# shibatch/rectdetect

Hardware: AMD Instinct MI355X
Metric: 1920x1080 frames/sec (higher is better)
Workload: dtype u8/i32/f32 (bit-exact integer + IEEE f32 stencil path)

## Files before the change

### rectdetect_amd/csrc/rd_k_poly.hip

```cpp
#include "rd_device.h"
#include "rd_kernels.h"

#include "rd_poly_scratch.h"
#include "rd_tidy_tile.h"

namespace {

using namespace rd;
using rdk::PolyScratch;
using rdk::PolyFrame;
#define RD_FRAME const PolyFrame &FRM = FRS.f[blockIdx.z]; const PolyScratch &s = FRM.ps

inline int cdiv(int a, int b) { return (a + b - 1) / b; }
const dim3 block2(64, 4);
inline dim3 grid2(int iw, int ih) { return dim3(cdiv(iw, 64), cdiv(ih, 4)); }
#define RD_XY const int x = blockIdx.x * 64 + threadIdx.x, y = blockIdx.y * 4 + threadIdx.y
#define SPARSE_GRID 512
#define SPARSE_LOOP(i, cnt) for (int i = blockIdx.x * blockDim.x + threadIdx.x; i < (cnt); i += gridDim.x * blockDim.x)

struct ls_rec { float x0, y0, x1, y1; int startIndex, endIndex, leftPtr, rightPtr, startCount, endCount, maxDist, polyid, npix, level; };
struct lsx_rec { long long mx00, mx01, mx11, my0, my1; short dx, dy, vx, vy; int d2, pad; };

typedef unsigned long long u64;
#define PT_M 6
#define TB_OUT (64 - 2 * PT_M)

__global__ __launch_bounds__(256) void k_mask_bits(const rdk::PolyFrames FRS, int iw, int ih, int wpr) {
  RD_FRAME;
  const int x = blockIdx.x * 64 + threadIdx.x, y = blockIdx.y * 4 + threadIdx.y;
  if (y >= ih) return;
  const bool in = x < iw;
  const int v = FRM.in[in ? y * iw + x : 0];
  const u64 m = __ballot(in && v != 0);
  u64 q = 0;
  if (FRM.ring_src != nullptr) {
    const bool ring = in && (y <= 1 || y >= ih - 2 || x <= 1 || x >= iw - 2);
    const int g = ring ? FRM.ring_src[y * iw + x] : 0;
    q = __ballot(g != 0);
  }
  if (threadIdx.x == 0) { s.sb[y * wpr + blockIdx.x] = m; s.rb[y * wpr + blockIdx.x] = q; }
}

__device__ __forceinline__ bitrow br_lane(bitrow a, int src_lane) {
  const unsigned a0 = (unsigned)a.lo, a1 = (unsigned)(a.lo >> 32), a2 = (unsigned)a.hi, a3 = (unsigned)(a.hi >> 32);
  const unsigned b0 = __shfl(a0, src_lane), b1 = __shfl(a1, src_lane), b2 = __shfl(a2, src_lane), b3 = __shfl(a3, src_lane);
  return br((u64)b0 | ((u64)b1 << 32), (u64)b2 | ((u64)b3 << 32));
}

__global__ __launch_bounds__(256) void k_tidy_bits(const rdk::PolyFrames FRS, int ring_const, int iw, int ih, int wpr) {
  RD_FRAME;
  const u64 *__restrict__ SB = FRM.in_bits != nullptr ? FRM.in_bits : s.sb;
  const u64 *__restrict__ RB = (FRM.in_bits == nullptr && FRM.ring_src != nullptr) ? s.rb : nullptr;
  if (blockIdx.x == 0 && blockIdx.y == 0 && threadIdx.x == 0) s.csync[0] = s.csync[0] + 1;
  const int lane = threadIdx.x & 63, wx = blockIdx.x * 4 + (threadIdx.x >> 6);
  if (wx >= wpr) return;
  constexpr int R = 64;
  const int x0 = wx * 64, y0 = blockIdx.y * TB_OUT;
  const int r = lane, y = y0 - PT_M + r;
  const bool yin = y >= 0 && y < ih;
  bitrow M = br(0, 0), RG = br(0, 0);
  if (yin) {
    const u64 *row = SB + (size_t)y * wpr + wx;
    const u64 W = wx > 0 ? row[-1] : 0ull, C = row[0], E = wx + 1 < wpr ? row[1] : 0ull;
    M = br((W >> 58) | (C << 6), (C >> 58) | (E << 6));
    if (RB != nullptr) {
      const u64 *rr = RB + (size_t)y * wpr + wx;
      const u64 W2 = wx > 0 ? rr[-1] : 0ull, C2 = rr[0], E2w = wx + 1 < wpr ? rr[1] : 0ull;
      RG = br((W2 >> 58) | (C2 << 6), (C2 >> 58) | (E2w << 6));
    }
  }
  const int b0 = PT_M - x0;
// ... 59 lines not shown
  const int lane = threadIdx.x & 63, y = blockIdx.x * 4 + (threadIdx.x >> 6);
  if (y >= ih) return;
  int run = 0;
  for (int w0 = 0; w0 < wpr; w0 += 64) {
    const int i = w0 + lane;
    const int c = i < wpr ? __popcll(s.tb[(size_t)y * wpr + i]) : 0;
    int inc = c;
#pragma unroll
    for (int o = 1; o < 64; o <<= 1) { const int t = __shfl_up(inc, o); if (lane >= o) inc += t; }
    if (i < wpr) s.pw[(size_t)y * wpr + i] = run + inc - c;
    run += __shfl(inc, 63);
  }
  if (lane == 0) s.rowsum[y] = run;
}

__device__ __forceinline__ int px_rank(const PolyScratch &s, int wpr, int qx, int qy) {
  const size_t wi = (size_t)qy * wpr + (qx >> 6);
  const u64 w = s.tb[wi];
  const int b = qx & 63;
  if (!((w >> b) & 1ull)) return -1;
  return s.rowbase[qy] + s.pw[wi] + __popcll(w & ((1ull << b) - 1ull));
}

#define CS_ROWS_PER_BLOCK 8
__global__ __launch_bounds__(256) void k_chain_scatter(const rdk::PolyFrames FRS, int iw, int ih, int wpr) {
  RD_FRAME;
  __shared__ int part[256];
  __shared__ int base[CS_ROWS_PER_BLOCK + 1];
  const int tid = threadIdx.x, ya = blockIdx.x * CS_ROWS_PER_BLOCK;
  int acc = 0;
  for (int i = tid; i < ya; i += 256) acc += s.rowsum[i];
  part[tid] = acc;
  __syncthreads();
  for (int o = 128; o > 0; o >>= 1) { if (tid < o) part[tid] += part[tid + o]; __syncthreads(); }
  if (tid == 0) {
    int run = part[0];
    for (int j = 0; j < CS_ROWS_PER_BLOCK; j++) {
      base[j] = run;
      if (ya + j < ih) { s.rowbase[ya + j] = run; run += s.rowsum[ya + j]; }
    }
    base[CS_ROWS_PER_BLOCK] = run;
    if (ya + CS_ROWS_PER_BLOCK >= ih) s.ctr[0] = run;
  }
  __syncthreads();
  for (int t = tid; t < CS_ROWS_PER_BLOCK * wpr; t += 256) {
    const int j = t / wpr, wx = t - j * wpr, y = ya + j;
    if (y >= ih) break;
    u64 w = s.tb[(size_t)y * wpr + wx];
    int rank = base[j] + s.pw[(size_t)y * wpr + wx];
    const int p = y * iw + wx * 64;
    while (w) {
      const int b = __ffsll((long long)w) - 1;
      w &= w - 1;
      s.pos[rank] = p + b; s.lab[rank] = rank; s.ends[rank] = 0;
      rank++;
    }
  }
}

#define CP_PER_BLOCK 8192
#define CP_K (CP_PER_BLOCK / 256)
__device__ __forceinline__ unsigned long long cp_word(unsigned gen, unsigned status, unsigned value) { return ((unsigned long long)(gen & 0xffffffu) << 40) | ((unsigned long long)status << 38) | value; }
template <int MODE>
__global__ __launch_bounds__(256) void k_compact1(const rdk::PolyFrames FRS, int n, int nblk, int size_thre, int init_ls) {
  RD_FRAME;
  static_assert(MODE == 1 || MODE == 2, "two call sites");
  int *__restrict__ pos = MODE == 2 ? s.live : nullptr;
  int *__restrict__ rank1 = MODE == 1 ? s.rootid : nullptr;
  const int *nptr = s.ctr;
  int *cnt = MODE == 1 ? s.ctr + 1 : s.ctr + 24;
  unsigned long long *state = s.cstate + (size_t)MODE * nblk;
  const int *genp = s.csync;
  ls_rec *ls = (MODE == 2 && init_ls) ? (ls_rec *)FRM.lslist : nullptr;
  if (MODE == 2 && ls != nullptr && blockIdx.x == 0 && threadIdx.x == 0) {
    ls_rec z = {};
    ls[0] = z;
    s.segaux[0] = -1; s.segaux[1] = 0x7fffffff;
    for (int k = 2; k < 24; k++) s.ctr[k] = 0;
    s.ctr[25] = 0;
  }
  __shared__ int wcount[CP_K * 4 + 1];
  __shared__ int s_excl;
  const int tid = threadIdx.x, lane = tid & 63, w = tid >> 6;
  const int b = blockIdx.x;
  if (nptr) n = *nptr;
  if (b * CP_PER_BLOCK >= n) { if (b == 0 && tid == 0 && cnt) *cnt = 0; return; }
  const unsigned gen = (unsigned)*genp;
  unsigned on = 0;
  if (MODE == 1) {
    int l[CP_K], sz[CP_K];
#pragma unroll
    for (int k = 0; k < CP_K; k++) { const int i = b * CP_PER_BLOCK + k * 256 + tid; const int q = i < n ? i : 0; l[k] = s.lab2[q]; sz[k] = s.size[q]; }
#pragma unroll
    for (int k = 0; k < CP_K; k++) { const int i = b * CP_PER_BLOCK + k * 256 + tid; if (i < n && l[k] == i && sz[k] > size_thre) on |= 1u << k; }
  } else {
    int l[CP_K];
#pragma unroll
    for (int k = 0; k < CP_K; k++) { const int i = b * CP_PER_BLOCK + k * 256 + tid; l[k] = s.lab2[i < n ? i : 0]; }
#pragma unroll
    for (int k = 0; k < CP_K; k++) l[k] = l[k] >= 0 ? s.rootid[l[k]] : 0;
#pragma unroll
    for (int k = 0; k < CP_K; k++) { const int i = b * CP_PER_BLOCK + k * 256 + tid; if (i < n) { s.id[i] = l[k]; if (l[k] != 0) on |= 1u << k; } }
  }
#pragma unroll
  for (int k = 0; k < CP_K; k++) { const unsigned long long m = __ballot((on >> k) & 1u); if (lane == 0) wcount[k * 4 + w] = __popcll(m); }
  __syncthreads();
  if (w == 0) {
    constexpr int CP_E = (CP_K * 4 + 63) / 64;
    int e[CP_E], c = 0;
#pragma unroll
    for (int q = 0; q < CP_E; q++) { e[q] = lane * CP_E + q < CP_K * 4 ? wcount[lane * CP_E + q] : 0; c += e[q]; }
    int inc = c;
#pragma unroll
    for (int o = 1; o < 64; o <<= 1) { const int t = __shfl_up(inc, o); if (lane >= o) inc += t; }
    int run = inc - c;
#pragma unroll
    for (int q = 0; q < CP_E; q++) { if (lane * CP_E + q < CP_K * 4) wcount[lane * CP_E + q] = run; run += e[q]; }
    const int total = __shfl(inc, 63);
    if (lane == 0) __hip_atomic_store(&state[b], cp_word(gen, b == 0 ? 2u : 1u, (unsigned)total), __ATOMIC_RELAXED, __HIP_MEMORY_SCOPE_AGENT);
    int excl = 0;
    for (int j = b - 1; j >= 0; j -= 64) {
      const int idx = j - lane;
      unsigned long long st;
      bool ready;
      int spins = 0;
      do {
        st = idx >= 0 ? __hip_atomic_load(&state[idx], __ATOMIC_RELAXED, __HIP_MEMORY_SCOPE_AGENT) : cp_word(gen, 2u, 0u);
        ready = (unsigned)(st >> 40) == (gen & 0xffffffu) && ((st >> 38) & 3ull) != 0ull;
        if (++spins > (1 << 24)) abort();
      } while (!__all(ready));
      const unsigned long long pm = __ballot(((st >> 38) & 3ull) == 2ull);
      const int upto = pm ? __ffsll((long long)pm) - 1 : 63;
      int v = lane <= upto ? (int)(st & 0x3fffffffffull) : 0;
#pragma unroll
      for (int o = 32; o > 0; o >>= 1) v += __shfl_xor(v, o);
      excl += v;
      if (pm) break;
    }
    if (lane == 0) {
      s_excl = excl;
      if (b > 0) __hip_atomic_store(&state[b], cp_word(gen, 2u, (unsigned)(excl + total)), __ATOMIC_RELAXED, __HIP_MEMORY_SCOPE_AGENT);
      if ((b + 1) * CP_PER_BLOCK >= n && cnt) *cnt = excl + total;
    }
  }
  __syncthreads();
  const int excl = s_excl;
#pragma unroll
  for (int k = 0; k < CP_K; k++) {
    const int i = b * CP_PER_BLOCK + k * 256 + tid;
    const bool o = (on >> k) & 1u;
    const unsigned long long m = __ballot(o);
    if (i >= n) continue;
    const int rank = excl + wcount[k * 4 + w] + __popcll(m & ((1ull << lane) - 1ull));
    if (o) { if (pos) pos[rank] = i; if (rank1) rank1[i] = rank + 1; }
  }
}

__global__ void k_chain_union(const rdk::PolyFrames FRS, int iw, int wpr) {
  RD_FRAME;
  const int cnt = s.ctr[0];
  SPARSE_LOOP(i, cnt) {
    const int p = s.pos[i];
    const int py = p / iw, px = p - py * iw;
    int nb[8], deg = 0;
#pragma unroll
    for (int k = 0; k < 8; k++) nb[k] = px_rank(s, wpr, px + nbr_dx(k), py + nbr_dy(k));
#pragma unroll
    for (int k = 0; k < 8; k++) { s.nbr[i * 8 + k] = nb[k]; deg += nb[k] >= 0; }
    s.flag2[i] = deg;
#pragma unroll
    for (int k = 0; k < 8; k++) if (nb[k] >= 0 && nb[k] < i) uf_union(s.lab, i, nb[k]);
  }
}

__global__ void k_flatten(const rdk::PolyFrames FRS, int which) {
  RD_FRAME;
  int *lab = which == 0 ? s.lab : s.lab2;
  int *ends = which == 0 ? s.ends : nullptr;
  const int *deg = s.flag2;
  int *size = which == 0 ? nullptr : s.size;
  const int cnt = s.ctr[0];
  for (int i0 = (blockIdx.x * blockDim.x + threadIdx.x) & ~63; i0 < cnt; i0 += gridDim.x * blockDim.x) {
    const int lane = threadIdx.x & 63, i = i0 + lane;
    int r = -1;
    if (i < cnt) {
      const int l = lab[i];
      r = l;
      if (l >= 0) { r = uf_find(lab, l); if (r != l) lab[i] = r; }
      if (ends != nullptr && deg[i] == 1) atomicAdd(&ends[r], 1);
    }
    if (size != nullptr) {
      const int prev = __shfl_up(r, 1);
      const bool start = lane == 0 || prev != r;
      const unsigned long long after = __ballot(start) & ~((2ull << lane) - 1ull);
      if (start && r >= 0) atomicAdd(&size[r], (after ? __ffsll((long long)after) - 1 : 64) - lane);
    }
  }
}

__global__ void k_find_ends0(const rdk::PolyFrames FRS) {
  RD_FRAME;
  const int cnt = s.ctr[0];
  SPARSE_LOOP(i, cnt) {
    int nb[8], lb[8], eb[8];
#pragma unroll
    for (int k = 0; k < 8; k++) nb[k] = s.nbr[i * 8 + k];
    const int li = s.lab[i], ei = s.ends[i];
#pragma unroll
    for (int k = 0; k < 8; k++) { const int j = nb[k] >= 0 ? nb[k] : i; lb[k] = s.lab[j]; eb[k] = s.ends[j]; }
    int a = i, b = i;
    const bool me = !(li == i && ei == 0);
    s.alive[i] = me ? 1 : 0;
    if (me) {
      int found = 0;
#pragma unroll
      for (int k = 0; k < 8; k++) {
        const bool living = nb[k] >= 0 && !(lb[k] == nb[k] && eb[k] == 0);
        if (living && found == 0) { a = nb[k]; found = 1; }
        else if (living && found == 1) { b = nb[k]; found = 2; }
      }
    }
    s.nx[0][i] = a; s.pv[0][i] = b;
  }
}

__global__ void k_find_ends0_flags(const rdk::PolyFrames FRS) {
  RD_FRAME;
  const int cnt = s.ctr[0];
  SPARSE_LOOP(i, cnt) {
    int f = 0;
    if (s.alive[i]) {
      const int a = s.nx[0][i], b = s.pv[0][i];
      if (a != i && s.nx[0][a] == i) f |= 1;
      if (b != i && s.pv[0][b] == i) f |= 2;
    }
    s.flag[i] = f;
  }
}

__global__ void k_find_ends1(const rdk::PolyFrames FRS, int page, int final) {
  RD_FRAME;
  const int cnt = s.ctr[0];
  const int *ni = s.nx[page], *pi = s.pv[page];
  int *no = s.nx[page ^ 1], *po = s.pv[page ^ 1];
  const int *fin = page == 0 ? s.flag : s.flag2;
  int *fout = page == 0 ? s.flag2 : s.flag;
  SPARSE_LOOP(i, cnt) {
    if (!s.alive[i]) { no[i] = i; po[i] = i; fout[i] = fin[i]; if (final) { s.num[0][i] = 0; s.link[0][i] = -1; } continue; }
    const int f0 = fin[i];
    bool revn = page == 0 ? (f0 & 1) != 0 : (f0 & 4) != 0;
    bool revp = page == 0 ? (f0 & 2) != 0 : (f0 & 8) != 0;
    int nn = ni[i], pp = pi[i];
    for (int h = 0; h < 8; h++) {
      const int nn2 = revn ? pi[nn] : ni[nn];
      const int pp2 = revp ? ni[pp] : pi[pp];
      int nf = fin[nn], pf = fin[pp];
      if (page != 0) { nf >>= 2; pf >>= 2; }
      revn = revn ? ((nf & 2) == 0) : ((nf & 1) != 0);
      revp = revp ? ((pf & 1) == 0) : ((pf & 2) != 0);
      nn = nn2; pp = pp2;
    }
    no[i] = nn; po[i] = pp;
    int f = f0;
    if (page == 0) { f &= 3; f |= revn ? 4 : 0; f |= revp ? 8 : 0; }
    else { f &= (3 << 2); f |= revn ? 1 : 0; f |= revp ? 2 : 0; }
    fout[i] = f;
    if (final) {
      int nb[8], al[8];
#pragma unroll
      for (int k = 0; k < 8; k++) nb[k] = s.nbr[i * 8 + k];
#pragma unroll
      for (int k = 0; k < 8; k++) al[k] = s.alive[nb[k] >= 0 ? nb[k] : i];
      int a = i, b = i, found = 0;
#pragma unroll
      for (int k = 0; k < 8; k++) {
        const bool living = nb[k] >= 0 && al[k] != 0;
        if (living && found == 0) { a = nb[k]; found = 1; }
        else if (living && found == 1) { b = nb[k]; found = 2; }
      }
      const int lk = nn < pp ? a : b;
      s.num[0][i] = lk == i ? 0 : 1; s.link[0][i] = lk;
    }
  }
}

__global__ void k_number(const rdk::PolyFrames FRS, int src, int init_sub) {
  RD_FRAME;
  const int cnt = s.ctr[0];
  const int *ni = s.num[src], *li = s.link[src];
  int *no = s.num[src ^ 1], *lo_ = s.link[src ^ 1];
  SPARSE_LOOP(i, cnt) {
    int n = ni[i], l = li[i];
    if (l != -1) {
      bool ok = true;
      for (int h = 0; h < 32; h++) {
        if (l < 0) { ok = false; break; }
        n += ni[l];
        l = li[l];
      }
      n = ok ? n : 0;
      l = ok ? l : -1;
    }
    no[i] = n;
    lo_[i] = l;
    if (init_sub) { s.lab2[i] = n == 0 ? -1 : i; s.size[i] = 0; s.rootid[i] = 0; }
  }
}

__global__ void k_sub_union(const rdk::PolyFrames FRS) {
  RD_FRAME;
  const int *__restrict__ number = s.num[1];
  const int cnt = s.ctr[0];
  SPARSE_LOOP(i, cnt) {
    const int a = number[i];
    if (a == 0) continue;
#pragma unroll
    for (int k = 0; k < 8; k++) {
      const int j = s.nbr[i * 8 + k];
      if (j < 0 || j > i) continue;
      const int b = number[j];
      if (b == 0) continue;
      const int d = a > b ? a - b : b - a;
      if (d <= 1) uf_union(s.lab2, i, j);
    }
  }
}

#define FITS(g, bytes) ((g) >= 0 && (long long)(bytes) > (long long)((g) + 1) * 56ll)

__device__ __forceinline__ void d_seg_clear(const rdk::PolyFrames &FRS, int lsbytes) {
  RD_FRAME;
  ls_rec *ls = (ls_rec *)FRM.lslist;
  const int K = s.ctr[1];
  const int maxrec = lsbytes / 56;
  SPARSE_LOOP(g, K + 1) {
    if (g >= maxrec) continue;
    ls_rec z = {};
    ls[g] = z;
    s.segaux[2 * g] = -1;
    s.segaux[2 * g + 1] = 0x7fffffff;
  }
  if (blockIdx.x == 0 && threadIdx.x == 0) { for (int k = 2; k < 24; k++) s.ctr[k] = 0; s.ctr[25] = 0; }
}
__global__ void k_seg_clear(const rdk::PolyFrames FRS, int lsbytes) { d_seg_clear(FRS, lsbytes); }

__device__ __forceinline__ void d_seg_pass0a(const rdk::PolyFrames &FRS, int lsbytes) {
  RD_FRAME;
  ls_rec *ls = (ls_rec *)FRM.lslist;
  const int *__restrict__ number = s.num[1];
  const int nlive = s.ctr[24];
  SPARSE_LOOP(j, nlive) {
    const int i = s.live[j];
    const int g = s.id[i];
    if (g == 0 || !FITS(g, lsbytes)) continue;
    const int n = number[i];
    if (n == 1) { atomicAdd(&ls[g].startCount, 1); atomicMax(&s.segaux[2 * g], i); }
    atomicAdd(&ls[g].npix, 1);
    atomicMax(&ls[g].endIndex, n);
  }
}
__global__ void k_seg_pass0a(const rdk::PolyFrames FRS, int lsbytes) { d_seg_pass0a(FRS, lsbytes); }

__device__ __forceinline__ void d_seg_pass0b(const rdk::PolyFrames &FRS, int lsbytes) {
  RD_FRAME;
  ls_rec *ls = (ls_rec *)FRM.lslist;
  const int *__restrict__ number = s.num[1];
  const int nlive = s.ctr[24];
  SPARSE_LOOP(j, nlive) {
    const int i = s.live[j];
    const int g = s.id[i];
    if (g == 0 || !FITS(g, lsbytes)) continue;
    if (number[i] != ls[g].endIndex) continue;
    if (ls[g].startCount == 1 && ls[g].npix >= 2) { atomicAdd(&ls[g].endCount, 1); atomicMin(&s.segaux[2 * g + 1], i); }
  }
}
__global__ void k_seg_pass0b(const rdk::PolyFrames FRS, int lsbytes) { d_seg_pass0b(FRS, lsbytes); }

__device__ __forceinline__ void d_seg_finish(const rdk::PolyFrames &FRS, int lsbytes, int iw) {
  RD_FRAME;
  ls_rec *ls = (ls_rec *)FRM.lslist;
  const int K = s.ctr[1];
  SPARSE_LOOP(g0, K) {
    const int g = g0 + 1;
    if (!FITS(g, lsbytes)) continue;
    const int sp = s.segaux[2 * g], ep = s.segaux[2 * g + 1];
    if (sp >= 0) { const int p = s.pos[sp]; ls[g].x0 = (float)(p % iw); ls[g].y0 = (float)(p / iw); }
    if (ls[g].startCount == 1 && ls[g].npix >= 2 && ep != 0x7fffffff) {
      const int p = s.pos[ep];
      ls[g].x1 = (float)(p % iw); ls[g].y1 = (float)(p / iw);
      ls[g].polyid = g;
    } else ls[g].polyid = 0;
  }
  if (blockIdx.x == 0 && threadIdx.x == 0) { const int top = lsbytes >= 57 ? (lsbytes - 1) / 56 - 1 : 0; *(int *)ls = K < top ? K : top; }
}
__global__ void k_seg_finish(const rdk::PolyFrames FRS, int lsbytes, int iw) { d_seg_finish(FRS, lsbytes, iw); }

__device__ __forceinline__ float dist2f(float vx, float vy, float wx, float wy) { return (vx - wx) * (vx - wx) + (vy - wy) * (vy - wy); }

__device__ __forceinline__ void d_split_move_dist(const rdk::PolyFrames &FRS, int lsbytes, int iw, int do_dist) {
  RD_FRAME;
  ls_rec *ls = (ls_rec *)FRM.lslist;
  const int *__restrict__ number = s.num[1];
  const int nlive = s.ctr[24];
  SPARSE_LOOP(j, nlive) {
    const int i = s.live[j];
    int g = s.id[i];
    if (g == 0 || !FITS(g, lsbytes) || ls[g].polyid == 0) continue;
    if (ls[g].endIndex < number[i]) { g = ls[g].rightPtr; s.id[i] = g; }
    if (!do_dist) continue;
    if (g == 0 || !FITS(g, lsbytes) || ls[g].polyid == 0) continue;
    const int p = s.pos[i], x = p % iw, y = p / iw;
    const float vx = (float)(int)ls[g].x0, vy = (float)(int)ls[g].y0, wx = (float)(int)ls[g].x1, wy = (float)(int)ls[g].y1;
    float cx, cy;
    const float l2 = dist2f(vx, vy, wx, wy);
    if (l2 <= 1e-4f) { cx = vx; cy = vy; }
    else {
      const float t = (((float)x - vx) * (wx - vx) + ((float)y - vy) * (wy - vy)) / l2;
      if (t < 0.0f) { cx = vx; cy = vy; }
      else if (t > 1.0f) { cx = wx; cy = wy; }
      else { cx = vx + t * (wx - vx); cy = vy + t * (wy - vy); }
    }
    const float a = cx - (float)x, b = cy - (float)y;
    int d = (int)((float)sqrt((double)a * (double)a + (double)b * (double)b) * 65536);
    d ^= pixel_rand(p, 0) & 0x1fff;
    s.dist[i] = d;
    atomicMax(&ls[g].maxDist, d);
  }
}
__global__ void k_split_move_dist(const rdk::PolyFrames FRS, int lsbytes, int iw, int do_dist) { d_split_move_dist(FRS, lsbytes, iw, do_dist); }

__device__ __forceinline__ void d_split_detect(const rdk::PolyFrames &FRS, int lsbytes, float minerror, int iw, int round) {
  RD_FRAME;
  const ls_rec *ls = (const ls_rec *)FRM.lslist;
  const int *__restrict__ number = s.num[1];
  const int nlive = s.ctr[24];
  SPARSE_LOOP(j, nlive) {
    const int i = s.live[j];
    const int g = s.id[i];
    if (g == 0 || !FITS(g, lsbytes)) continue;
    const ls_rec r = ls[g];
    if (r.polyid == 0) continue;
    if (r.endIndex - r.startIndex < 3) continue;
    if (r.startCount > 1 || r.endCount > 1) continue;
    const int md = r.maxDist;
    if (s.dist[i] != md) continue;
    if (md < (int)(minerror * 65536)) continue;
    if ((float)md < (minerror * 3 * 65536) && (float)md * (float)md / dist2f(r.x0, r.y0, r.x1, r.y1) < 100000.0f) continue;
    const int p = s.pos[i], x = p % iw, y = p / iw;
    if (dist2f((float)x, (float)y, r.x0, r.y0) < 1) continue;
    if (dist2f((float)x, (float)y, r.x1, r.y1) < 1) continue;
    const int c = atomicAdd(&s.ctr[2 + round], 1);
    int *e = s.cand + (size_t)c * 8;
    e[0] = i; e[1] = g; e[2] = number[i]; e[3] = md; e[4] = r.endIndex; e[5] = r.rightPtr;
    e[6] = __float_as_int(r.x1); e[7] = __float_as_int(r.y1);
  }
}
__global__ void k_split_detect(const rdk::PolyFrames FRS, int lsbytes, float minerror, int iw, int round) { d_split_detect(FRS, lsbytes, minerror, iw, round); }

__device__ __forceinline__ void d_split_apply(const rdk::PolyFrames &FRS, int lsbytes, int iw, int round) {
  RD_FRAME;
  ls_rec *ls = (ls_rec *)FRM.lslist;
  const int C = s.ctr[2 + round];
  const int base = *(const int *)ls;
  SPARSE_LOOP(c, C) {
    const int *e = s.cand + (size_t)c * 8;
    const int i = e[0], g = e[1];
    int rank = 0;
    bool last = true;
    for (int k = 0; k < C; k++) {
      const int *f = s.cand + (size_t)k * 8;
      if (f[0] < i) rank++;
      if (f[1] == g && f[0] > i) last = false;
    }
    const int gn = base + 1 + rank;
    if (!FITS(gn, lsbytes)) continue;
    const int p = s.pos[i], x = p % iw, y = p / iw;
    ls_rec nr = {};
    nr.startIndex = e[2]; nr.endIndex = e[4];
    nr.x0 = (float)x; nr.y0 = (float)y; nr.x1 = __int_as_float(e[6]); nr.y1 = __int_as_float(e[7]);
    nr.leftPtr = g; nr.rightPtr = e[5];
    nr.maxDist = 0; nr.polyid = ls[g].polyid; nr.level = e[3];
    ls[gn] = nr;
    if (last) {
      ls[g].endIndex = e[2]; ls[g].x1 = (float)x; ls[g].y1 = (float)y; ls[g].rightPtr = gn; ls[g].maxDist = 0;
      if (e[5] != 0) ls[e[5]].leftPtr = gn;
    }
  }
// ... 148 lines not shown
  const float l2 = dist2f(vx, vy, wx, wy);
  if (l2 <= 1e-4f) { cx = vx; cy = vy; }
  else {
    const float t = (((float)x - vx) * (wx - vx) + ((float)y - vy) * (wy - vy)) / l2;
    if (t < 0.0f) { cx = vx; cy = vy; }
    else if (t > 1.0f) { cx = wx; cy = wy; }
    else { cx = vx + t * (wx - vx); cy = vy + t * (wy - vy); }
  }
  const float a = cx - (float)x, b = cy - (float)y;
  int d = (int)((float)sqrt((double)a * (double)a + (double)b * (double)b) * 65536);
  d ^= rnd13;
  dreg = d;
  atomicMax(&L.rec[g].maxDist, d);
  return make_int2(pk, dreg);
}

__device__ __noinline__ void pp_detect(pp_lds &L, int pk, int xyv, int dreg, float minerror, const int *live, int j) {
  const int g = pk & 0x7ff;
  const ls_rec r = L.rec[g];
  if (r.polyid == 0) return;
  if (r.endIndex - r.startIndex < 3) return;
  if (r.startCount > 1 || r.endCount > 1) return;
  const int md = r.maxDist;
  if (dreg != md) return;
  if (md < (int)(minerror * 65536)) return;
  if ((float)md < (minerror * 3 * 65536) && (float)md * (float)md / dist2f(r.x0, r.y0, r.x1, r.y1) < 100000.0f) return;
  const int x = xyv & 0xffff, y = xyv >> 16;
  if (dist2f((float)x, (float)y, r.x0, r.y0) < 1) return;
  if (dist2f((float)x, (float)y, r.x1, r.y1) < 1) return;
  const int c = atomicAdd(&L.ncand, 1);
  if (c >= PP_MAXCAND) { L.fail = 1; return; }
  int *e = L.cand + c * 8;
  e[0] = live[j]; e[1] = g; e[2] = (int)((unsigned)pk >> 11); e[3] = md; e[4] = r.endIndex; e[5] = r.rightPtr;
  e[6] = __float_as_int(r.x1); e[7] = __float_as_int(r.y1);
}

__device__ __noinline__ void pp_moments(pp_lds &L, int pk, int xyv, int n) {
  const int g = pk & 0x7ff;
  if (g <= 0 || n < g || L.rec[g].polyid == 0) return;
  const int vx = (xyv & 0xffff) - (int)rintf(L.rec[g].x0), vy = (xyv >> 16) - (int)rintf(L.rec[g].y0);
  const int ay = vx * L.sx[g].vx + vy * L.sx[g].vy;
  const int ax0 = vx * L.sx[g].dx + vy * L.sx[g].dy;
  const int ax1 = L.sx[g].d2;
  atomicAdd((unsigned long long *)&L.sx[g].mx00, (unsigned long long)(long long)rintf((float)ax0 * (float)ax0));
  atomicAdd((unsigned long long *)&L.sx[g].mx01, (unsigned long long)(long long)rintf((float)ax0 * (float)ax1));
  atomicAdd((unsigned long long *)&L.sx[g].mx11, (unsigned long long)(long long)rintf((float)ax1 * (float)ax1));
  atomicAdd((unsigned long long *)&L.sx[g].my0, (unsigned long long)(long long)rintf((float)ax0 * (float)ay));
  atomicAdd((unsigned long long *)&L.sx[g].my1, (unsigned long long)(long long)rintf((float)ax1 * (float)ay));
}

__global__ __launch_bounds__(PP_T) void k_poly_persistent(const rdk::PolyFrames FRS, int lsbytes, float minerror, int iw) {
  RD_FRAME;
  ls_rec *ls = (ls_rec *)FRM.lslist;
  const int *__restrict__ number = s.num[1];
  extern __shared__ __attribute__((aligned(16))) char pp_raw[];
  pp_lds &L = *(pp_lds *)pp_raw;
  const int tid = threadIdx.x;
  const int nlive = s.ctr[24], K = s.ctr[1];
  const int maxrec = lsbytes / 56;
  if (tid == 0) s.ctr[39] = (int)wall_clock64();
  if (nlive > PP_T * PP_PX || K >= PP_MAXSEG - 1 || K >= maxrec - 1) { if (tid == 0) s.ctr[25] = 1; return; }

  int pk[PP_PX], xy[PP_PX], dreg[PP_PX], rnd[PP_PX / 2];
#define PP_ID(k) (pk[k] & 0x7ff)
#define PP_NUM(k) ((int)((unsigned)pk[k] >> 11))
#define PP_CI(k) (s.live[tid + (k) * PP_T])
#define PP_SEQ __builtin_amdgcn_sched_barrier(0)
  {
    int cc[PP_PX];
#pragma unroll
    for (int k = 0; k < PP_PX; k++) { const int j = tid + k * PP_T; cc[k] = s.live[j < nlive ? j : 0]; }
#pragma unroll
    for (int k = 0; k < PP_PX; k++) { const int j = tid + k * PP_T; if (j >= nlive) cc[k] = 0; }
#pragma unroll
    for (int k = 0; k < PP_PX; k++) { xy[k] = s.pos[cc[k]]; pk[k] = s.id[cc[k]]; dreg[k] = number[cc[k]]; }
#pragma unroll
    for (int k = 0; k < PP_PX; k++) {
      const int j = tid + k * PP_T;
      const int p = xy[k];
      pk[k] = j < nlive ? (pk[k] | (dreg[k] << 11)) : 0;
      xy[k] = j < nlive ? ((p % iw) | ((p / iw) << 16)) : 0;
      dreg[k] = 0;
      if ((k & 1) == 0) rnd[k >> 1] = 0;
      rnd[k >> 1] |= (j < nlive ? (pixel_rand(p, 0) & 0x1fff) : 0) << (16 * (k & 1));
      PP_SEQ;
    }
  }
  for (int g = tid; g < PP_MAXSEG; g += PP_T) L.done[g] = 0;
  for (int g = tid; g <= K; g += PP_T) { ls_rec z = {}; L.rec[g] = z; L.start_i[g] = -1; L.end_i[g] = 0x7fffffff; }
  if (tid == 0) { L.ncand = 0; L.count = K; L.fail = 0; L.progress[0] = 0; L.progress[1] = 0; }
  __syncthreads();

  if (tid == 0) s.ctr[40] = (int)wall_clock64();
#pragma unroll
  for (int k = 0; k < PP_PX; k++) {
    const int g = PP_ID(k);
    if (g != 0) {
      if (PP_NUM(k) == 1) { atomicAdd(&L.rec[g].startCount, 1); atomicMax(&L.start_i[g], PP_CI(k)); }
      atomicAdd(&L.rec[g].npix, 1);
      atomicMax(&L.rec[g].endIndex, PP_NUM(k));
    }
    PP_SEQ;
  }
  __syncthreads();
#pragma unroll
  for (int k = 0; k < PP_PX; k++) {
    const int g = PP_ID(k);
// ... 131 lines not shown
        const float e1 = sqrtf((wx - u0) * (wx - u0) + (wy - u1) * (wy - u1));
        if (e0 > 10 && e1 > 10) { wx = (v2 + u0) * 0.5f; wy = (v3 + u1) * 0.5f; }
      }
      L.rec[g].x1 = wx; L.rec[g].y1 = wy; L.rec[h].x0 = wx; L.rec[h].y0 = wy;
      L.done[g] = 1;
      L.progress[iter & 1] = 1;
    }
    __syncthreads();
    if (!L.progress[iter & 1]) break;
  }

  if (tid == 0) s.ctr[44] = (int)wall_clock64();
  if (tid == 0) { ls_rec z = {}; ls[0] = z; *(int *)ls = n; if (L.fail) s.ctr[25] = 1; }
  for (int g = tid + 1; g <= n; g += PP_T) ls[g] = L.rec[g];
#pragma unroll
  for (int k = 0; k < PP_PX; k++) if (tid + k * PP_T < nlive) s.id[PP_CI(k)] = PP_ID(k);
  if (tid == 0) s.ctr[45] = (int)wall_clock64();
}

__global__ void k_scatter_ids(const rdk::PolyFrames FRS) {
  RD_FRAME;
  int *ids = FRM.ids;
  const int nlive = s.ctr[24];
  SPARSE_LOOP(j, nlive) { const int i = s.live[j]; ids[s.pos[i]] = s.id[i]; }
}

__global__ __launch_bounds__(256) void k_poly_handoff(const rdk::PolyFrames FRS, int records) {
  RD_FRAME;
  const int *__restrict__ ls = (const int *)FRM.lslist;
  int *__restrict__ pack = FRM.pack;
  const int n = ls[0];
  const int m = (n + 1 < records ? n + 1 : records) * 14;
  const int t = blockIdx.x * blockDim.x + threadIdx.x;
  if (t < 32) pack[t] = s.ctr[t];
  for (int i = t; i < m; i += gridDim.x * blockDim.x) pack[64 + i] = ls[i];
}

template <typename T> T *dalloc(size_t n) { void *p = nullptr; if (hipMalloc(&p, n * sizeof(T)) != hipSuccess) return nullptr; return (T *)p; }

}

namespace rdk {

PolyScratch *poly_scratch_create(int iw, int ih) {
  PolyScratch *ps = new PolyScratch();
  const size_t N = (size_t)iw * ih;
  ps->cap = (int)N;
  const size_t NWORDS = (size_t)cdiv(iw, 64) * ih + 8;
  ps->sb = dalloc<unsigned long long>(NWORDS); ps->rb = dalloc<unsigned long long>(NWORDS); ps->tb = dalloc<unsigned long long>(NWORDS);
  ps->pw = dalloc<int>(NWORDS); ps->rowsum = dalloc<int>(ih + 8); ps->rowbase = dalloc<int>(ih + 8);
  ps->cstate = dalloc<unsigned long long>(3 * (N / CP_PER_BLOCK + 2)); ps->csync = dalloc<int>(4);
  ps->pos = dalloc<int>(N); ps->nbr = dalloc<int>(N * 8);
  ps->lab = dalloc<int>(N); ps->alive = dalloc<int>(N); ps->ends = dalloc<int>(N);
  for (int k = 0; k < 2; k++) { ps->nx[k] = dalloc<int>(N); ps->pv[k] = dalloc<int>(N); ps->num[k] = dalloc<int>(N); ps->link[k] = dalloc<int>(N); }
  ps->flag = dalloc<int>(N); ps->flag2 = dalloc<int>(N);
  ps->lab2 = dalloc<int>(N); ps->size = dalloc<int>(N); ps->rootid = dalloc<int>(N); ps->id = dalloc<int>(N); ps->dist = dalloc<int>(N + 2);
  ps->cand = dalloc<int>(N * 8 / 4 + 64);
  ps->ctr = dalloc<int>(64);
  ps->lsx = dalloc<lsx_rec>(N * 16 / 56 + 2);
  ps->segaux = dalloc<int>(2 * (N * 16 / 56 + 2));
  ps->live = dalloc<int>(N);
  (void)hipMemset(ps->ctr, 0, 64 * sizeof(int));
  (void)hipMemset(ps->cstate, 0, 3 * (N / CP_PER_BLOCK + 2) * sizeof(unsigned long long));
  (void)hipMemset(ps->csync, 0, 4 * sizeof(int));
  (void)hipStreamSynchronize(0);
  return ps;
}

const int *poly_scratch_counters(const PolyScratch *ps) { return ps->ctr; }

static_assert(PP_MAXSEG <= (1 << 11), "a record id must fit the id field of the packed per-pixel word");
void poly_limits(int out[4]) { out[0] = PP_T * PP_PX; out[1] = PP_MAXSEG; out[2] = PP_MAXCAND; out[3] = 11; }

void poly_scratch_destroy(PolyScratch *ps) {
  if (!ps) return;
  void *all[] = { ps->sb, ps->rb, ps->tb, ps->pw, ps->rowsum, ps->rowbase, ps->cstate, ps->csync, ps->pos, ps->nbr, ps->lab, ps->alive, ps->ends, ps->nx[0], ps->nx[1], ps->pv[0], ps->pv[1],
                  ps->num[0], ps->num[1], ps->link[0], ps->link[1], ps->flag, ps->flag2, ps->lab2, ps->size, ps->rootid, ps->id, ps->dist, ps->cand, ps->ctr, ps->lsx, ps->segaux, ps->live };
  for (void *p : all) if (p) (void)hipFree(p);
  delete ps;
}

void polyline(hipStream_t st, const PolyFrame *frames_host, int nb, int lslist_bytes, int ring_const, float minerror, int sizeThre, int iw, int ih, int mode) {
  const PolyFrames frames = pack_frames(frames_host, nb);
  const int N = iw * ih;
  const int maxrec = lslist_bytes / 56;
  const dim3 sg(SPARSE_GRID, 1, nb), sb(256);

  const int wpr = cdiv(iw, 64);
  for (int z = 0; z < nb; z++) {
    if ((frames_host[z].in_bits == nullptr) != (frames_host[0].in_bits == nullptr)) { fprintf(stderr, "polyline: the frames of one launch mix bit-plane and int-plane input\n"); abort(); }
    if (frames_host[z].in_bits != nullptr && frames_host[z].ring_src != nullptr) { fprintf(stderr, "polyline: a frame hands over a bit plane AND a ring source (the ring is only read from int planes)\n"); abort(); }
  }
  if (frames_host[0].in_bits == nullptr) hipLaunchKernelGGL(k_mask_bits, dim3(wpr, cdiv(ih, 4), nb), dim3(64, 4), 0, st, frames, iw, ih, wpr);
  hipLaunchKernelGGL(k_tidy_bits, dim3(cdiv(wpr, 4), cdiv(ih, TB_OUT), nb), dim3(256), 0, st, frames, ring_const, iw, ih, wpr);
  hipLaunchKernelGGL(k_row_prefix, dim3(cdiv(ih, 4), 1, nb), dim3(256), 0, st, frames, ih, wpr);
  hipLaunchKernelGGL(k_chain_scatter, dim3(cdiv(ih, CS_ROWS_PER_BLOCK), 1, nb), dim3(256), 0, st, frames, iw, ih, wpr);
  const int nblk = cdiv(N, CP_PER_BLOCK);
  const dim3 cg(nblk, 1, nb);

  hipLaunchKernelGGL(k_chain_union, sg, sb, 0, st, frames, iw, wpr);
  hipLaunchKernelGGL(k_flatten, sg, sb, 0, st, frames, 0);
  hipLaunchKernelGGL(k_find_ends0, sg, sb, 0, st, frames);
  hipLaunchKernelGGL(k_find_ends0_flags, sg, sb, 0, st, frames);
  for (int r = 0; r < 4; r++) hipLaunchKernelGGL(k_find_ends1, sg, sb, 0, st, frames, r & 1, r == 3 ? 1 : 0);
  for (int r = 0; r < 3; r++) hipLaunchKernelGGL(k_number, sg, sb, 0, st, frames, r & 1, r == 2 ? 1 : 0);

  hipLaunchKernelGGL(k_sub_union, sg, sb, 0, st, frames);
  hipLaunchKernelGGL(k_flatten, sg, sb, 0, st, frames, 1);
  hipLaunchKernelGGL(k_compact1<1>, cg, dim3(256), 0, st, frames, N, nblk, sizeThre, 0);
  hipLaunchKernelGGL(k_compact1<2>, cg, dim3(256), 0, st, frames, N, nblk, 0, mode == 1 ? 1 : 0);

  if (mode == 1) {
    static std::atomic<unsigned> lds_set{0};
    set_max_lds_once((const void *)k_poly_persistent, (int)sizeof(pp_lds), lds_set);
    hipLaunchKernelGGL(k_poly_persistent, dim3(1, 1, nb), dim3(PP_T), sizeof(pp_lds), st, frames, lslist_bytes, minerror, iw);
    return;
  }

  hipLaunchKernelGGL(k_seg_clear, sg, sb, 0, st, frames, lslist_bytes);
  hipLaunchKernelGGL(k_seg_pass0a, sg, sb, 0, st, frames, lslist_bytes);
  hipLaunchKernelGGL(k_seg_pass0b, sg, sb, 0, st, frames, lslist_bytes);
  hipLaunchKernelGGL(k_seg_finish, sg, sb, 0, st, frames, lslist_bytes, iw);

  for (int r = 0; r < 15; r++) {
    hipLaunchKernelGGL(k_split_move_dist, sg, sb, 0, st, frames, lslist_bytes, iw, 1);
    hipLaunchKernelGGL(k_split_detect, sg, sb, 0, st, frames, lslist_bytes, minerror, iw, r);
    hipLaunchKernelGGL(k_split_apply, sg, sb, 0, st, frames, lslist_bytes, iw, r);
    hipLaunchKernelGGL(k_split_commit, dim3(1, 1, nb), dim3(64), 0, st, frames, r);
  }
  hipLaunchKernelGGL(k_split_move_dist, sg, sb, 0, st, frames, lslist_bytes, iw, 0);

  hipLaunchKernelGGL(k_refine0, sg, sb, 0, st, frames, maxrec);
  hipLaunchKernelGGL(k_refine1, sg, sb, 0, st, frames, maxrec, iw);
  hipLaunchKernelGGL(k_refine2, sg, sb, 0, st, frames, maxrec);
  hipLaunchKernelGGL(k_refine3, dim3(1, 1, nb), dim3(1024), 0, st, frames, maxrec);
}

void polyline_handoff(hipStream_t st, const PolyFrame *frames_host, int nb, int records) {
  const PolyFrames frames = pack_frames(frames_host, nb);
  int g = cdiv(records * 14, 256);
  if (g > 128) g = 128;
  hipLaunchKernelGGL(k_poly_handoff, dim3(g < 1 ? 1 : g, 1, nb), dim3(256), 0, st, frames, records);
}

void polyline_ids(hipStream_t st, const PolyFrame *frames_host, int nb, int n) {
  const PolyFrames frames = pack_frames(frames_host, nb);
  for (int z = 0; z < nb; z++) (void)hipMemsetAsync(frames_host[z].ids, 0, sizeof(int) * (size_t)n, st);
  hipLaunchKernelGGL(k_scatter_ids, dim3(SPARSE_GRID, 1, nb), dim3(256), 0, st, frames);
}

}
```

### rectdetect_amd/csrc/rd_poly_scratch.h

```cpp
#pragma once

namespace rdk {

struct PolyScratch {
  int cap;
  unsigned long long *sb, *rb;
  unsigned long long *tb;
  int *pw, *rowsum, *rowbase;
  unsigned long long *cstate;
  int *csync;
  int *pos;
  int *nbr;
  int *lab, *alive, *ends;
  int *nx[2], *pv[2], *flag, *flag2;
  int *num[2], *link[2];
  int *lab2, *size, *rootid, *id, *dist;
  int *cand;
  int *ctr;
  void *lsx;
  int *segaux;
  int *live;
};

struct PolyFrame {
  PolyScratch ps;
  const int *in;
  const unsigned long long *in_bits;
  const int *ring_src;
  void *lslist;
  int *ids;
  const int *boundary;
  int *table, *claim, *tlist;
  int *probes;
  int *pack;
  const int *rflags;
  int *post_scratch;
  int *post_out;
};
#define RD_POST_MAXC 1024

#define RD_MAXB 8
struct PolyFrames { PolyFrame f[RD_MAXB]; };
inline PolyFrames pack_frames(const PolyFrame *frames, int nb) {
  PolyFrames r;
  for (int z = 0; z < RD_MAXB; z++) r.f[z] = frames[z < nb ? z : 0];
  return r;
}

}
```

Before: 3168.

## Compact surviving pixels by component size and pack end-search records into int2

```diff
diff --git a/rectdetect_amd/csrc/rd_k_poly.hip b/rectdetect_amd/csrc/rd_k_poly.hip
--- a/rectdetect_amd/csrc/rd_k_poly.hip
+++ b/rectdetect_amd/csrc/rd_k_poly.hip
@@ -17,6 +17,7 @@
 #define RD_XY const int x = blockIdx.x * 64 + threadIdx.x, y = blockIdx.y * 4 + threadIdx.y
 #define SPARSE_GRID 512
 #define SPARSE_LOOP(i, cnt) for (int i = blockIdx.x * blockDim.x + threadIdx.x; i < (cnt); i += gridDim.x * blockDim.x)
+#define SURV_LOOP(i) for (int j_ = blockIdx.x * blockDim.x + threadIdx.x, ns_ = s.ctr[26]; j_ < ns_; j_ += gridDim.x * blockDim.x) if (const int i = s.surv[j_]; true)
 
 struct ls_rec { float x0, y0, x1, y1; int startIndex, endIndex, leftPtr, rightPtr, startCount, endCount, maxDist, polyid, npix, level; };
 struct lsx_rec { long long mx00, mx01, mx11, my0, my1; short dx, dy, vx, vy; int d2, pad; };
@@ -182,7 +183,7 @@
     while (w) {
       const int b = __ffsll((long long)w) - 1;
       w &= w - 1;
-      s.pos[rank] = p + b; s.lab[rank] = rank; s.ends[rank] = 0;
+      s.pos[rank] = p + b; s.lab[rank] = rank; s.ends[rank] = 0; s.size[rank] = 0;
       rank++;
     }
   }
@@ -194,11 +195,11 @@
 template <int MODE>
 __global__ __launch_bounds__(256) void k_compact1(const rdk::PolyFrames FRS, int n, int nblk, int size_thre, int init_ls) {
   RD_FRAME;
-  static_assert(MODE == 1 || MODE == 2, "two call sites");
-  int *__restrict__ pos = MODE == 2 ? s.live : nullptr;
+  static_assert(MODE == 0 || MODE == 1 || MODE == 2, "three call sites");
+  int *__restrict__ pos = MODE == 2 ? s.live : MODE == 0 ? s.surv : nullptr;
   int *__restrict__ rank1 = MODE == 1 ? s.rootid : nullptr;
   const int *nptr = s.ctr;
-  int *cnt = MODE == 1 ? s.ctr + 1 : s.ctr + 24;
+  int *cnt = MODE == 1 ? s.ctr + 1 : MODE == 2 ? s.ctr + 24 : s.ctr + 26;
   unsigned long long *state = s.cstate + (size_t)MODE * nblk;
   const int *genp = s.csync;
   ls_rec *ls = (MODE == 2 && init_ls) ? (ls_rec *)FRM.lslist : nullptr;
@@ -217,7 +218,15 @@
   if (b * CP_PER_BLOCK >= n) { if (b == 0 && tid == 0 && cnt) *cnt = 0; return; }
   const unsigned gen = (unsigned)*genp;
   unsigned on = 0;
-  if (MODE == 1) {
+  if (MODE == 0) {
+    int l[CP_K];
+#pragma unroll
+    for (int k = 0; k < CP_K; k++) { const int i = b * CP_PER_BLOCK + k * 256 + tid; l[k] = s.lab[i < n ? i : 0]; }
+#pragma unroll
+    for (int k = 0; k < CP_K; k++) l[k] = s.size[l[k]];
+#pragma unroll
+    for (int k = 0; k < CP_K; k++) { const int i = b * CP_PER_BLOCK + k * 256 + tid; if (i < n) { if (l[k] > size_thre) on |= 1u << k; else s.lab2[i] = -1; } }
+  } else if (MODE == 1) {
     int l[CP_K], sz[CP_K];
 #pragma unroll
     for (int k = 0; k < CP_K; k++) { const int i = b * CP_PER_BLOCK + k * 256 + tid; const int q = i < n ? i : 0; l[k] = s.lab2[q]; sz[k] = s.size[q]; }
@@ -308,18 +317,19 @@
   int *lab = which == 0 ? s.lab : s.lab2;
   int *ends = which == 0 ? s.ends : nullptr;
   const int *deg = s.flag2;
-  int *size = which == 0 ? nullptr : s.size;
-  const int cnt = s.ctr[0];
-  for (int i0 = (blockIdx.x * blockDim.x + threadIdx.x) & ~63; i0 < cnt; i0 += gridDim.x * blockDim.x) {
-    const int lane = threadIdx.x & 63, i = i0 + lane;
+  int *size = s.size;
+  const int cnt = which == 0 ? s.ctr[0] : s.ctr[26];
+  for (int j0 = (blockIdx.x * blockDim.x + threadIdx.x) & ~63; j0 < cnt; j0 += gridDim.x * blockDim.x) {
+    const int lane = threadIdx.x & 63, j = j0 + lane;
     int r = -1;
-    if (i < cnt) {
+    if (j < cnt) {
+      const int i = which == 0 ? j : s.surv[j];
       const int l = lab[i];
       r = l;
       if (l >= 0) { r = uf_find(lab, l); if (r != l) lab[i] = r; }
       if (ends != nullptr && deg[i] == 1) atomicAdd(&ends[r], 1);
     }
-    if (size != nullptr) {
+    {
       const int prev = __shfl_up(r, 1);
       const bool start = lane == 0 || prev != r;
       const unsigned long long after = __ballot(start) & ~((2ull << lane) - 1ull);
@@ -330,8 +340,7 @@
 
 __global__ void k_find_ends0(const rdk::PolyFrames FRS) {
   RD_FRAME;
-  const int cnt = s.ctr[0];
-  SPARSE_LOOP(i, cnt) {
+  SURV_LOOP(i) {
     int nb[8], lb[8], eb[8];
 #pragma unroll
     for (int k = 0; k < 8; k++) nb[k] = s.nbr[i * 8 + k];
@@ -350,100 +359,92 @@
         else if (living && found == 1) { b = nb[k]; found = 2; }
       }
     }
-    s.nx[0][i] = a; s.pv[0][i] = b;
-  }
-}
-
+    s.ne[1][i] = make_int2(a, b);
+  }
+}
+
+#define NE_IDX 0x3fffffff
+#define NE_BIT(v) (((v) >> 30) & 1)
 __global__ void k_find_ends0_flags(const rdk::PolyFrames FRS) {
   RD_FRAME;
-  const int cnt = s.ctr[0];
-  SPARSE_LOOP(i, cnt) {
-    int f = 0;
+  const int2 *__restrict__ raw = s.ne[1];
+  SURV_LOOP(i) {
+    int2 r = raw[i];
     if (s.alive[i]) {
-      const int a = s.nx[0][i], b = s.pv[0][i];
-      if (a != i && s.nx[0][a] == i) f |= 1;
-      if (b != i && s.pv[0][b] == i) f |= 2;
-    }
-    s.flag[i] = f;
+      const int a = r.x, b = r.y;
+      if (a != i && raw[a].x == i) r.x |= 1 << 30;
+      if (b != i && raw[b].y == i) r.y |= 1 << 30;
+    }
+    s.ne[0][i] = r;
   }
 }
 
 __global__ void k_find_ends1(const rdk::PolyFrames FRS, int page, int final) {
   RD_FRAME;
-  const int cnt = s.ctr[0];
-  const int *ni = s.nx[page], *pi = s.pv[page];
-  int *no = s.nx[page ^ 1], *po = s.pv[page ^ 1];
-  const int *fin = page == 0 ? s.flag : s.flag2;
-  int *fout = page == 0 ? s.flag2 : s.flag;
-  SPARSE_LOOP(i, cnt) {
-    if (!s.alive[i]) { no[i] = i; po[i] = i; fout[i] = fin[i]; if (final) { s.num[0][i] = 0; s.link[0][i] = -1; } continue; }
-    const int f0 = fin[i];
-    bool revn = page == 0 ? (f0 & 1) != 0 : (f0 & 4) != 0;
-    bool revp = page == 0 ? (f0 & 2) != 0 : (f0 & 8) != 0;
-    int nn = ni[i], pp = pi[i];
+  const int2 *__restrict__ rin = s.ne[page];
+  int2 *__restrict__ rout = s.ne[page ^ 1];
+  SURV_LOOP(i) {
+    const int2 me = rin[i];
+    if (!s.alive[i]) { rout[i] = me; if (final) s.nl[0][i] = make_int2(0, -1); continue; }
+    bool revn = NE_BIT(me.x) != 0, revp = NE_BIT(me.y) != 0;
+    int nn = me.x & NE_IDX, pp = me.y & NE_IDX;
     for (int h = 0; h < 8; h++) {
-      const int nn2 = revn ? pi[nn] : ni[nn];
-      const int pp2 = revp ? ni[pp] : pi[pp];
-      int nf = fin[nn], pf = fin[pp];
-      if (page != 0) { nf >>= 2; pf >>= 2; }
-      revn = revn ? ((nf & 2) == 0) : ((nf & 1) != 0);
-      revp = revp ? ((pf & 1) == 0) : ((pf & 2) != 0);
-      nn = nn2; pp = pp2;
-    }
-    no[i] = nn; po[i] = pp;
-    int f = f0;
-    if (page == 0) { f &= 3; f |= revn ? 4 : 0; f |= revp ? 8 : 0; }
-    else { f &= (3 << 2); f |= revn ? 1 : 0; f |= revp ? 2 : 0; }
-    fout[i] = f;
-    if (final) {
-      int nb[8], al[8];
-#pragma unroll
-      for (int k = 0; k < 8; k++) nb[k] = s.nbr[i * 8 + k];
-#pragma unroll
-      for (int k = 0; k < 8; k++) al[k] = s.alive[nb[k] >= 0 ? nb[k] : i];
-      int a = i, b = i, found = 0;
-#pragma unroll
-      for (int k = 0; k < 8; k++) {
-        const bool living = nb[k] >= 0 && al[k] != 0;
-        if (living && found == 0) { a = nb[k]; found = 1; }
-        else if (living && found == 1) { b = nb[k]; found = 2; }
-      }
-      const int lk = nn < pp ? a : b;
-      s.num[0][i] = lk == i ? 0 : 1; s.link[0][i] = lk;
-    }
-  }
-}
-
-__global__ void k_number(const rdk::PolyFrames FRS, int src, int init_sub) {
-  RD_FRAME;
-  const int cnt = s.ctr[0];
-  const int *ni = s.num[src], *li = s.link[src];
-  int *no = s.num[src ^ 1], *lo_ = s.link[src ^ 1];
-  SPARSE_LOOP(i, cnt) {
-    int n = ni[i], l = li[i];
+      const int2 rn = rin[nn], rp = rin[pp];
+      nn = (revn ? rn.y : rn.x) & NE_IDX;
+      pp = (revp ? rp.x : rp.y) & NE_IDX;
+      revn = revn ? NE_BIT(rn.y) == 0 : NE_BIT(rn.x) != 0;
+      revp = revp ? NE_BIT(rp.x) == 0 : NE_BIT(rp.y) != 0;
+    }
+    if (!final) { rout[i] = make_int2(nn | (revn ? 1 << 30 : 0), pp | (revp ? 1 << 30 : 0)); continue; }
+    int nb[8], al[8];
+#pragma unroll
+    for (int k = 0; k < 8; k++) nb[k] = s.nbr[i * 8 + k];
+#pragma unroll
+    for (int k = 0; k < 8; k++) al[k] = s.alive[nb[k] >= 0 ? nb[k] : i];
+    int a = i, b = i, found = 0;
+#pragma unroll
+    for (int k = 0; k < 8; k++) {
+      const bool living = nb[k] >= 0 && al[k] != 0;
+      if (living && found == 0) { a = nb[k]; found = 1; }
+      else if (living && found == 1) { b = nb[k]; found = 2; }
+    }
+    const int lk = nn < pp ? a : b;
+    s.nl[0][i] = make_int2(lk == i ? 0 : 1, lk);
+  }
+}
+
+__global__ void k_number(const rdk::PolyFrames FRS, int src, int last) {
+  RD_FRAME;
+  const int2 *__restrict__ in = s.nl[src];
+  int2 *__restrict__ out = s.nl[src ^ 1];
+  SURV_LOOP(i) {
+    const int2 me = in[i];
+    int n = me.x, l = me.y;
     if (l != -1) {
       bool ok = true;
       for (int h = 0; h < 32; h++) {
         if (l < 0) { ok = false; break; }
-        n += ni[l];
-        l = li[l];
+        const int2 r = in[l];
+        n += r.x;
+        if (r.y == l && r.x == 0) break;
+        l = r.y;
       }
       n = ok ? n : 0;
       l = ok ? l : -1;
     }
-    no[i] = n;
-    lo_[i] = l;
-    if (init_sub) { s.lab2[i] = n == 0 ? -1 : i; s.size[i] = 0; s.rootid[i] = 0; }
+    if (!last) { out[i] = make_int2(n, l); continue; }
+    s.num[i] = n;
+    s.lab2[i] = n == 0 ? -1 : i; s.size[i] = 0; s.rootid[i] = 0;
   }
 }
 
 __global__ void k_sub_union(const rdk::PolyFrames FRS) {
   RD_FRAME;
-  const int *__restrict__ number = s.num[1];
+  const int *__restrict__ number = s.num;
   const int cnt = s.ctr[0];
   SPARSE_LOOP(i, cnt) {
+    if (s.lab2[i] < 0) continue;
     const int a = number[i];
-    if (a == 0) continue;
 #pragma unroll
     for (int k = 0; k < 8; k++) {
       const int j = s.nbr[i * 8 + k];
@@ -477,7 +478,7 @@
 __device__ __forceinline__ void d_seg_pass0a(const rdk::PolyFrames &FRS, int lsbytes) {
   RD_FRAME;
   ls_rec *ls = (ls_rec *)FRM.lslist;
-  const int *__restrict__ number = s.num[1];
+  const int *__restrict__ number = s.num;
   const int nlive = s.ctr[24];
   SPARSE_LOOP(j, nlive) {
     const int i = s.live[j];
@@ -494,7 +495,7 @@
 __device__ __forceinline__ void d_seg_pass0b(const rdk::PolyFrames &FRS, int lsbytes) {
   RD_FRAME;
   ls_rec *ls = (ls_rec *)FRM.lslist;
-  const int *__restrict__ number = s.num[1];
+  const int *__restrict__ number = s.num;
   const int nlive = s.ctr[24];
   SPARSE_LOOP(j, nlive) {
     const int i = s.live[j];
@@ -530,7 +531,7 @@
 __device__ __forceinline__ void d_split_move_dist(const rdk::PolyFrames &FRS, int lsbytes, int iw, int do_dist) {
   RD_FRAME;
   ls_rec *ls = (ls_rec *)FRM.lslist;
-  const int *__restrict__ number = s.num[1];
+  const int *__restrict__ number = s.num;
   const int nlive = s.ctr[24];
   SPARSE_LOOP(j, nlive) {
     const int i = s.live[j];
@@ -562,7 +563,7 @@
 __device__ __forceinline__ void d_split_detect(const rdk::PolyFrames &FRS, int lsbytes, float minerror, int iw, int round) {
   RD_FRAME;
   const ls_rec *ls = (const ls_rec *)FRM.lslist;
-  const int *__restrict__ number = s.num[1];
+  const int *__restrict__ number = s.num;
   const int nlive = s.ctr[24];
   SPARSE_LOOP(j, nlive) {
     const int i = s.live[j];
@@ -817,7 +818,7 @@
 __global__ __launch_bounds__(PP_T) void k_poly_persistent(const rdk::PolyFrames FRS, int lsbytes, float minerror, int iw) {
   RD_FRAME;
   ls_rec *ls = (ls_rec *)FRM.lslist;
-  const int *__restrict__ number = s.num[1];
+  const int *__restrict__ number = s.num;
   extern __shared__ __attribute__((aligned(16))) char pp_raw[];
   pp_lds &L = *(pp_lds *)pp_raw;
   const int tid = threadIdx.x;
@@ -1055,7 +1056,8 @@
   ps->cstate = dalloc<unsigned long long>(3 * (N / CP_PER_BLOCK + 2)); ps->csync = dalloc<int>(4);
   ps->pos = dalloc<int>(N); ps->nbr = dalloc<int>(N * 8);
   ps->lab = dalloc<int>(N); ps->alive = dalloc<int>(N); ps->ends = dalloc<int>(N);
-  for (int k = 0; k < 2; k++) { ps->nx[k] = dalloc<int>(N); ps->pv[k] = dalloc<int>(N); ps->num[k] = dalloc<int>(N); ps->link[k] = dalloc<int>(N); }
+  for (int k = 0; k < 2; k++) { ps->ne[k] = dalloc<int2>(N); ps->nl[k] = dalloc<int2>(N); }
+  ps->num = dalloc<int>(N); ps->surv = dalloc<int>(N);
   ps->flag = dalloc<int>(N); ps->flag2 = dalloc<int>(N);
   ps->lab2 = dalloc<int>(N); ps->size = dalloc<int>(N); ps->rootid = dalloc<int>(N); ps->id = dalloc<int>(N); ps->dist = dalloc<int>(N + 2);
   ps->cand = dalloc<int>(N * 8 / 4 + 64);
@@ -1077,8 +1079,8 @@
 
 void poly_scratch_destroy(PolyScratch *ps) {
   if (!ps) return;
-  void *all[] = { ps->sb, ps->rb, ps->tb, ps->pw, ps->rowsum, ps->rowbase, ps->cstate, ps->csync, ps->pos, ps->nbr, ps->lab, ps->alive, ps->ends, ps->nx[0], ps->nx[1], ps->pv[0], ps->pv[1],
-                  ps->num[0], ps->num[1], ps->link[0], ps->link[1], ps->flag, ps->flag2, ps->lab2, ps->size, ps->rootid, ps->id, ps->dist, ps->cand, ps->ctr, ps->lsx, ps->segaux, ps->live };
+  void *all[] = { ps->sb, ps->rb, ps->tb, ps->pw, ps->rowsum, ps->rowbase, ps->cstate, ps->csync, ps->pos, ps->nbr, ps->lab, ps->alive, ps->ends, ps->ne[0], ps->ne[1], ps->nl[0], ps->nl[1],
+                  ps->num, ps->surv, ps->flag, ps->flag2, ps->lab2, ps->size, ps->rootid, ps->id, ps->dist, ps->cand, ps->ctr, ps->lsx, ps->segaux, ps->live };
   for (void *p : all) if (p) (void)hipFree(p);
   delete ps;
 }
@@ -1086,8 +1088,12 @@
 void polyline(hipStream_t st, const PolyFrame *frames_host, int nb, int lslist_bytes, int ring_const, float minerror, int sizeThre, int iw, int ih, int mode) {
   const PolyFrames frames = pack_frames(frames_host, nb);
   const int N = iw * ih;
+  if (N > NE_IDX) { fprintf(stderr, "polyline: %dx%d: compact indices must stay below 2^30 (the records of the end search keep a bit beside them)\n", iw, ih); abort(); }
   const int maxrec = lslist_bytes / 56;
   const dim3 sg(SPARSE_GRID, 1, nb), sb(256);
+  int svb = cdiv(N, 128 * 256);
+  svb = svb < 32 ? 32 : svb > SPARSE_GRID ? SPARSE_GRID : svb;
+  const dim3 sv(svb, 1, nb);
 
   const int wpr = cdiv(iw, 64);
   for (int z = 0; z < nb; z++) {
@@ -1103,13 +1109,14 @@
 
   hipLaunchKernelGGL(k_chain_union, sg, sb, 0, st, frames, iw, wpr);
   hipLaunchKernelGGL(k_flatten, sg, sb, 0, st, frames, 0);
-  hipLaunchKernelGGL(k_find_ends0, sg, sb, 0, st, frames);
-  hipLaunchKernelGGL(k_find_ends0_flags, sg, sb, 0, st, frames);
-  for (int r = 0; r < 4; r++) hipLaunchKernelGGL(k_find_ends1, sg, sb, 0, st, frames, r & 1, r == 3 ? 1 : 0);
-  for (int r = 0; r < 3; r++) hipLaunchKernelGGL(k_number, sg, sb, 0, st, frames, r & 1, r == 2 ? 1 : 0);
+  hipLaunchKernelGGL(k_compact1<0>, cg, dim3(256), 0, st, frames, N, nblk, sizeThre, 0);
+  hipLaunchKernelGGL(k_find_ends0, sv, sb, 0, st, frames);
+  hipLaunchKernelGGL(k_find_ends0_flags, sv, sb, 0, st, frames);
+  for (int r = 0; r < 4; r++) hipLaunchKernelGGL(k_find_ends1, sv, sb, 0, st, frames, r & 1, r == 3 ? 1 : 0);
+  for (int r = 0; r < 3; r++) hipLaunchKernelGGL(k_number, sv, sb, 0, st, frames, r & 1, r == 2 ? 1 : 0);
 
   hipLaunchKernelGGL(k_sub_union, sg, sb, 0, st, frames);
-  hipLaunchKernelGGL(k_flatten, sg, sb, 0, st, frames, 1);
+  hipLaunchKernelGGL(k_flatten, sv, sb, 0, st, frames, 1);
   hipLaunchKernelGGL(k_compact1<1>, cg, dim3(256), 0, st, frames, N, nblk, sizeThre, 0);
   hipLaunchKernelGGL(k_compact1<2>, cg, dim3(256), 0, st, frames, N, nblk, 0, mode == 1 ? 1 : 0);
 
diff --git a/rectdetect_amd/csrc/rd_poly_scratch.h b/rectdetect_amd/csrc/rd_poly_scratch.h
--- a/rectdetect_amd/csrc/rd_poly_scratch.h
+++ b/rectdetect_amd/csrc/rd_poly_scratch.h
@@ -12,9 +12,12 @@
   int *pos;
   int *nbr;
   int *lab, *alive, *ends;
-  int *nx[2], *pv[2], *flag, *flag2;
-  int *num[2], *link[2];
+  int2 *ne[2];
+  int *flag, *flag2;
+  int2 *nl[2];
+  int *num;
   int *lab2, *size, *rootid, *id, *dist;
+  int *surv;
   int *cand;
   int *ctr;
   void *lsx;
@@ -41,6 +44,7 @@
 
 #define RD_MAXB 8
 struct PolyFrames { PolyFrame f[RD_MAXB]; };
+static_assert(sizeof(PolyFrames) + 64 + 256 <= 4096, "the descriptors travel by value: with a launch's other arguments (64 bytes at the most) and the 256 bytes the compiler appends they must fit 4 KB of kernel arguments");
 inline PolyFrames pack_frames(const PolyFrame *frames, int nb) {
   PolyFrames r;
   for (int z = 0; z < RD_MAXB; z++) r.f[z] = frames[z < nb ? z : 0];
```

After: 3383, median of 6. +6.8%, better.
